# LilYau350/Variance-Aware-Weight

Hardware: AMD Instinct MI355X
Metric: training images/sec (higher is better)
Workload: dtype bf16; 1 GPU; DiT-B/4, 4x32x32 latents, 1000 classes; Trainer.train_step: q_sample + fwd + lambda-weighted MSE + bwd + AdamW + EMA; global batch 256 = 256 per GPU; global_batch=256, per_gpu_batch=256, parallelism=dp1, weight_type=lambda, hip_graph=False

## Files before the change

### include/vaw_hip.h

```cpp
#ifndef VAW_HIP_H
#define VAW_HIP_H
#include <stdint.h>

#ifdef __cplusplus
extern "C" {
#endif

typedef enum { VAW_OK = 0, VAW_ERR_INVALID = -1, VAW_ERR_LAUNCH = -2, VAW_ERR_UNSUPPORTED = -3 } vaw_status;
typedef enum { VAW_F32 = 0, VAW_BF16 = 1,
               VAW_FP8 = 2, VAW_BF8 = 3 ,
               VAW_F64 = 4  } vaw_dtype;
typedef void* vaw_stream;

int vaw_version(void);
const char* vaw_last_error_string(void);


int vaw_qsample_fwd(const float* x0, const float* noise, const int64_t* t, const float* tab_a, const float* tab_s,
                    int num_timesteps, float* x_t, int B, int64_t per_sample, vaw_stream stream);

int vaw_mix_rows(const float* x, const float* y, const float* ca, const float* cb, float* out, int B,
                 int64_t per_sample, vaw_stream stream);

int vaw_wmse_fwd(const float* model_out, const float* x0, const float* noise, const float* ca, const float* cb,
// ... 235 lines not shown
    int split;
    int xcd_parts;
    int grid_x, grid_y, grid_z, block;
    int64_t lds_bytes;
    int reduce;
    int rowsum_mode;
    int colsum_mode;
    int64_t colsum_rows;
    int64_t workspace_floats_used;
    int launches;
    int status;
} vaw_gemm_launch;
int vaw_gemm_plan(vaw_dtype dt, int a_kmajor, int b_kmajor, int64_t M, int64_t N, int64_t K, int64_t lda, int64_t ldb,
                  int64_t ldc, int64_t A, int64_t B, int64_t C, const vaw_epilogue* epi_host, int64_t workspace_floats,
                  const vaw_gemm_knobs* knobs, vaw_gemm_launch* out);

typedef struct {
    int epi_kind;
    int a_e5m2;
    int c_fp8, c_e5m2;
    int ntw;
    int tiles_m, tiles_n;
    int nk;
    int split;
    int grid, block;
    int64_t lds_bytes;
    int colsum_mode;
    int64_t colsum_rows;
    int64_t workspace_floats_used;
    int launches;
// ... 259 lines not shown
```

### variance-aware-weight_amd/_lib.py

```python
import ctypes as C
import os

import torch

_HERE = os.path.dirname(os.path.abspath(__file__))
LIB_PATH = os.environ.get("VAW_HIP_LIB") or os.path.join(_HERE, "libvaw_hip.so")

F32, BF16, FP8, BF8 = 0, 1, 2, 3
F64 = 4
TORCH_DTYPE = {F32: torch.float32, BF16: torch.bfloat16}

_p, _i, _l, _f, _d = C.c_void_p, C.c_int, C.c_int64, C.c_float, C.c_double


class Epilogue(C.Structure):
    _fields_ = [("bias", _p), ("act", _i), ("aux_in", _p), ("aux_out", _p), ("gate", _p), ("gate_ld", _l),
                ("resid", _p), ("rowadd", _p), ("rows_per_batch", _i), ("alpha", _f), ("beta", _f), ("out_f32", _i),
                ("colsum_out", _p), ("colsum_beta", _f), ("resid_is_act", _i), ("rowsum_a_out", _p), ("rowsum_a_beta", _f),
                ("colsum_partial_out", _p), ("colsum_rows_out", C.POINTER(C.c_int64))]


class AttnDesc(C.Structure):
    _fields_ = [("B", _i), ("H", _i), ("T", _i), ("hd", _i), ("q_sb", _l), ("q_sh", _l), ("q_st", _l), ("q_sd", _l),
                ("o_sb", _l), ("o_sh", _l), ("o_st", _l), ("o_sd", _l), ("scale", _f)]
# ... 25 lines not shown
                ("xcd_parts", _i), ("grid_x", _i), ("grid_y", _i), ("grid_z", _i), ("block", _i), ("lds_bytes", _l), ("reduce", _i),
                ("rowsum_mode", _i), ("colsum_mode", _i), ("colsum_rows", _l), ("workspace_floats_used", _l), ("launches", _i),
                ("status", _i)]


class Conv3x3Launch(C.Structure):
    _fields_ = [("variant", _i), ("ntw", _i), ("epi_kind", _i), ("transposed", _i), ("M", _l), ("N", _l), ("K", _l), ("split", _i),
                ("xcd_parts", _i), ("grid_x", _i), ("grid_y", _i), ("block", _i), ("lds_bytes", _l), ("reduce", _i), ("bias_grad", _i),
                ("colsum_mode", _i), ("colsum_rows", _l), ("workspace_floats_used", _l), ("launches", _i), ("status", _i)]


class GemmFp8Launch(C.Structure):
    _fields_ = [("epi_kind", _i), ("a_e5m2", _i), ("c_fp8", _i), ("c_e5m2", _i), ("ntw", _i), ("tiles_m", _i), ("tiles_n", _i), ("nk", _i),
                ("split", _i), ("grid", _i), ("block", _i), ("lds_bytes", _l), ("colsum_mode", _i), ("colsum_rows", _l),
                ("workspace_floats_used", _l), ("launches", _i), ("status", _i)]


class DitWsPlan(C.Structure):
    _fields_ = [("records", _i), ("colsum_sets", _i), ("own_dy", _i), ("Bk", _i), ("block_bytes", _l), ("block_stat_bytes", _l),
                ("shared_bytes", _l), ("colsum_bytes", _l), ("scratch_bytes", _l), ("cond_bytes", _l), ("total", _l)]


class CastColsumLaunch(C.Structure):
    _fields_ = [("grid_x", _i), ("block", _i), ("rows_per_lane", _i), ("bytes_read", _l), ("bytes_written", _l)]


ATTN_FWD, ATTN_BWD, ATTN_BWD_COLSUM = range(3)
(AV_ROWWISE, AV_FWD_T64, AV_FWD_G1, AV_FWD_G2, AV_FWD_BIG, AV_BWD_T64, AV_BWD_G1, AV_BWD_G2, AV_BWD_BIG_NT2,
 AV_BWD_BIG_NT4) = range(10)
AV_NAMES = ("rowwise", "fwd_t64", "fwd_g1", "fwd_g2", "fwd_big", "bwd_t64", "bwd_g1", "bwd_g2", "bwd_big_nt2", "bwd_big_nt4")
# ... 105 lines not shown
    "vaw_uncast_bf16": [_p, _p, _l, _f, _p],
    "vaw_wgrad_grouped": [_i, _i, _p, _l, _f, _p, _i, _p, _l, _p],
    "vaw_fp8_quantize": [_i, _i, _p, _l, _l, _l, _p, _l, _p, _l, _p, _p, _l, _p],
    "vaw_fp8_quantize_delayed": [_i, _i, _p, _l, _l, _l, _p, _l, _p, _l, _p, _p],
    "vaw_fp8_scale_update": [_p, _l, _p],
    "vaw_fp8_quantize_delayed_batched": [_i, _p, _p, _i, _p],
    "vaw_gemm_fp8": [_i, _l, _l, _l, _p, _l, _p, _p, _l, _p, _p, _l, C.POINTER(Epilogue), _p, _i, _p, _l, _p],
    "vaw_gemm_fp8_plan": [_i, _l, _l, _l, _l, _l, _l, _l, _l, _l, _l, _l, C.POINTER(Epilogue), _l, _i, _l, _l, _i, C.POINTER(GemmFp8Launch)],
    "vaw_fp8_transpose": [_p, _l, _l, _l, _p, _l, _p],
    "vaw_ln_modulate_fwd_fp8": [_p, _p, _p, _l, _p, _p, _i, _p, _p, _i, _i, _i, _f, _p],
    "vaw_gate_bwd_fp8": [_p, _p, _p, _l, _p, _p, _i, _p, _l, _p, _i, _i, _i, _p, _l, _p],
    "vaw_row_plan": [_i, _i, _l, _l, _l, _l, _l, _l, C.POINTER(RowLaunch)],
    "vaw_attn_plan": [_i, _i, C.POINTER(AttnDesc), _l, _l, _l, _l, _l, _l, _l, C.POINTER(AttnLaunch)],
    "vaw_gn_plan": [_i, _i, _i, _i, _i, _i, C.POINTER(GnLaunch)],
    "vaw_gemm_plan": [_i, _i, _i, _l, _l, _l, _l, _l, _l, _l, _l, _l, C.POINTER(Epilogue), _l, C.POINTER(GemmKnobs), C.POINTER(GemmLaunch)],
    "vaw_conv3x3_plan": [_i, _i, _l, _l, _l, _l, _i, _i, _i, _i, _i, C.POINTER(Epilogue), _l, _l, C.POINTER(GemmKnobs), _i, C.POINTER(Conv3x3Launch)],
    "vaw_dit_ws_plan": [_i, _i, _i, _i, _i, _i, _i, _i, _i, _i, _i, C.POINTER(DitWsPlan)],
    "vaw_latent_qsample": [_p, _p, _p, _p, _p, _p, _i, _f, _f, _p, _p, _p, _i, _l, _p],
    "vaw_wmse_fwd_t": [_p, _p, _p, _p, _p, _p, _p, _i, _p, _p, _f, _i, _l, _p],
    "vaw_wmse_bwd_t": [_p, _p, _p, _p, _p, _p, _p, _i, _p, _f, _p, _i, _l, _p],
    "vaw_ln_modulate_bwd_cast": [_i, _p, _p, _p, _p, _p, _l, _p, _p, _p, _p, _l, _i, _i, _i, _p, _l, _p, _p],
    "vaw_silu_bwd_cast": [_p, _p, _p, _p, _l, _p],
    "vaw_cast_colsum_plan": [_l, _l, _l, _l, _l, _l, _l, C.POINTER(CastColsumLaunch)],
    "vaw_cast_colsum_bf16": [_p, _l, _p, _l, _l, _l, _p, _f, _p],
    "vaw_row_sqnorms": [_p, _l, _i, _p, _p],
    "vaw_pairwise_ksmallest": [_p, _l, _p, _l, _i, _p, _p, _i, _p, _p, _l, _p],
    "vaw_ksmallest_merge": [_p, _l, _i, _i, _l, _l, _p, _p],
    "vaw_pairwise_within": [_p, _l, _p, _l, _i, _p, _p, _p, _i, _p, _i, _p, _p, _p],
    "vaw_pairwise_polysum": [_p, _l, _p, _l, _i, _p, _p, _i, _d, _d, _i, _i, _p, _p, _l, _p],
    "vaw_pairwise_count_within": [_p, _l, _p, _l, _i, _p, _p, _p, _i, _p, _p, _p, _l, _p],
# ... 64 lines not shown
        L.vaw_debug_force_generic_gemm.argtypes = [_i]
        L.vaw_debug_force_generic_gemm.restype = None
        L.vaw_debug_gemm_tile.argtypes = [_i]
        L.vaw_debug_gemm_tile.restype = None
        if hasattr(L, "vaw_gemm_default_knobs"):
            L.vaw_gemm_default_knobs.argtypes = [C.POINTER(GemmKnobs)]
            L.vaw_gemm_default_knobs.restype = None
        if hasattr(L, "vaw_debug_gn_flat"):
            L.vaw_debug_gn_flat.argtypes = [_i]
            L.vaw_debug_gn_flat.restype = None
        L.vaw_p8_set_reserved_cus.argtypes = [_i]
        L.vaw_p8_set_reserved_cus.restype = None
        if hasattr(L, "vaw_debug_wgrad_engine"):
            L.vaw_debug_wgrad_engine.argtypes = [_i]
            L.vaw_debug_wgrad_engine.restype = None
        L.vaw_debug_cu_hog.argtypes = [_i, _i, _p]
        L.vaw_debug_cu_hog.restype = _i
        _lib = L
    return _lib


def exported_symbols():
    return sorted(list(_PROTOS) + ["vaw_version", "vaw_last_error_string", "vaw_colsum_workspace_floats",
                                   "vaw_sumsq_workspace_floats", "vaw_groupnorm_workspace_floats", "vaw_wgrad_grouped_desc_bytes",
                                   "vaw_conv3x3_wgrad_small_workspace_floats", "vaw_row_bwd_workspace_floats",
                                   "vaw_fp8_quantize_workspace_floats", "vaw_p8_set_reserved_cus", "vaw_debug_wgrad_engine", "vaw_reduce_rows_batched_desc_bytes", "vaw_fp8_quantize_batched_desc_bytes",
                                   "vaw_gemm_default_knobs", "vaw_dropout_bits_words", "vaw_pairwise_workspace_bytes", "vaw_rk_partial_count",
                                   "vaw_pairwise_polysum_workspace_bytes", "vaw_pairwise_count_workspace_bytes"])


STEP_FUSED = os.environ.get("VAW_STEP_FUSED", "1") != "0"
ROWS_FWD_FUSED = os.environ.get("VAW_ROWS_FWD_FUSED", "1") != "0"


def check(rc, what):
    if rc != 0:
        raise VawError(f"{what} failed ({rc}): {lib().vaw_last_error_string().decode()}")


def stream_ptr():
    return torch.cuda.current_stream().cuda_stream
# ... 11 lines not shown
```

### variance-aware-weight_amd/csrc/gemm_plan.h

```cpp
#pragma once
#include "gemm_epi.h"

typedef vaw_gemm_knobs GemmKnobs;
GemmKnobs& vaw_gemm_knobs_state();
int vaw_p8_cus_available();

struct P8Plan {
    bool use;
    int ntw, split, grid;
};
P8Plan vaw_p8_plan(int64_t M, int64_t N, int64_t K, bool plain_f32, bool want_colsum, int64_t ws_floats, int force, int cus);

inline int pick_split(int64_t tiles, int64_t K, int64_t MN, int64_t ws_floats, bool plain_f32) {
    if (!plain_f32 || ws_floats <= 0) return 1;
    int64_t s = 512 / tiles;
    if (s > K / 256) s = K / 256;
    if (s > ws_floats / MN) s = ws_floats / MN;
    if (s > 64) s = 64;
    return s < 2 ? 1 : (int)s;
}
inline int no_empty_split(int nk, int split) {
    if (split <= 1) return 1;
    const int per = (nk + split - 1) / split;
    return (nk + per - 1) / per;
}

inline int xcd_parts_for(const GemmKnobs& k, int split) { return (k.xcdsplit && (split == 2 || split == 4 || split == 8)) ? 8 / split : 0; }

constexpr int64_t vaw_lds_t128(int bkt) { return (8 * 128 * bkt > 64 * 132 * 4 ? 8 * 128 * bkt : 64 * 132 * 4) + 4 * 128 * 4; }
constexpr int64_t vaw_lds_ring256() { return 4 * 4 * (128 * 32 * 2) + 8 * 256 * 4; }
constexpr int64_t vaw_lds_p8(int ntw) { return 2 * (4 + ntw) * 8192 + 32768; }
constexpr int64_t vaw_lds_sm(int mb, int nb, int stages) { return (int64_t)stages * (mb + nb) * 8192; }
constexpr int64_t vaw_lds_pd(int ntw) { return 3 * (2 + ntw) * 8192 + 8 * 2048; }
constexpr int64_t vaw_lds_ws(int ntw) { return 3 * (2 + ntw) * 8192; }
constexpr int64_t vaw_lds_generic() { return 2 * 16 * 144 * 4; }

inline EpiDev vaw_epi_dev(const vaw_epilogue* ep, const GemmKnobs& k) {
    EpiDev e{};
    e.alpha = 1.f;
    if (ep) {
        e.bias = ep->bias; e.act = ep->act; e.aux_in = ep->aux_in; e.aux_out = ep->aux_out; e.gate = ep->gate;
        e.gate_ld = ep->gate_ld; e.resid = ep->resid; e.rowadd = ep->rowadd; e.rpb = ep->rows_per_batch;
        e.alpha = ep->alpha; e.beta = ep->beta; e.out_f32 = ep->out_f32; e.resid_act = ep->resid_is_act;
    }
    if (e.rpb <= 0) e.rpb = 1;
    e.debug = k.debug;
// ... 4 lines not shown
```

### variance-aware-weight_amd/csrc/gemm_plan.hip

```cpp
#include <stdlib.h>

#include "gemm_plan.h"

extern "C" void vaw_gemm_default_knobs(vaw_gemm_knobs* k) {
    *k = vaw_gemm_knobs{};
    k->tile = -1;
    k->xcdsplit = k->epi = k->nt_aux = 1;
    k->sm_max_m = 8192;
    k->ws_loaders = 4;
    k->cus = 256;
}
GemmKnobs& vaw_gemm_knobs_state() {
    static GemmKnobs state = [] {
        static const struct { const char* env; int GemmKnobs::*field; } kEnv[] = {
            {"VAW_GEMM_BIG", &GemmKnobs::tile}, {"VAW_GEMM_BK", &GemmKnobs::bk}, {"VAW_GEMM_PD", &GemmKnobs::pd}, {"VAW_GEMM_WS", &GemmKnobs::ws},
            {"VAW_GEMM_XCDSPLIT", &GemmKnobs::xcdsplit}, {"VAW_SM_MAX_M", &GemmKnobs::sm_max_m}, {"VAW_SM_WIDE_M", &GemmKnobs::sm_wide_m},
            {"VAW_SM_NB", &GemmKnobs::sm_nb}, {"VAW_SM_STAGES", &GemmKnobs::sm_stages}, {"VAW_WS_LOADERS", &GemmKnobs::ws_loaders},
            {"VAW_GEMM_EPI", &GemmKnobs::epi}, {"VAW_GEMM_DEBUG", &GemmKnobs::debug}, {"VAW_P8_NT", &GemmKnobs::p8_nt}, {"VAW_P8_NT_AUX", &GemmKnobs::nt_aux}};
        GemmKnobs k;
        vaw_gemm_default_knobs(&k);
        for (const auto& e : kEnv)
            if (const char* v = getenv(e.env)) k.*e.field = atoi(v);
        k.ws_loaders = k.ws_loaders == 8 ? 8 : 4;
        k.p8_nt = k.p8_nt == 1;
// ... 219 lines not shown
    }
    const bool fused = p.rowsum_mode == VAW_GS_FUSED;
    p.reduce = p.split == 1 ? VAW_GR_NONE : !e.out_f32 ? VAW_GR_BF16 : fused ? VAW_GR_F32_ROWSUM : VAW_GR_F32;
    p.workspace_floats_used = (p.split > 1 ? (int64_t)p.split * M * N : 0) + (fused ? (int64_t)p.split * M : 0) +
                              (p.colsum_mode == VAW_GC_FOLD ? p.colsum_rows * N : 0);
    p.launches += (p.reduce != VAW_GR_NONE) + (fused && p.split == 1) + (p.colsum_mode == VAW_GC_FOLD);
    if (p.rowsum_mode == VAW_GS_SEPARATE && !a_kmajor && (rc = colsum_pass(p, dt, K, M, lda, A, ws)) != VAW_OK) return rc;
    if (p.colsum_mode == VAW_GC_SEPARATE && (rc = colsum_pass(p, e.out_f32 ? VAW_F32 : dt, M, N, ldc, C, ws)) != VAW_OK) return rc;
    *out = p;
    VAW_CHECK_ARG(!cs_part || p.colsum_rows <= *ep->colsum_rows_out, "gemm: colsum_partial_out holds %ld rows, this launch writes %ld",
                  (long)*ep->colsum_rows_out, (long)p.colsum_rows);
    VAW_CHECK_ARG(p.rowsum_mode != VAW_GS_SEPARATE || !a_kmajor, "gemm: rowsum_a_out is defined for a_kmajor = 0 (weight-gradient layout) only");
    VAW_CHECK_ARG(p.workspace_floats_used <= ws, "gemm: this launch needs a workspace of %ld floats, it has %ld", (long)p.workspace_floats_used,
                  (long)ws);
    out->status = p.status = VAW_OK;
    return VAW_OK;
}

extern "C" int vaw_conv3x3_plan(vaw_dtype dt, int mode, int64_t act, int64_t act2, int64_t w, int64_t out, int B, int H, int W, int Ci,
                                int Co, const vaw_epilogue* ep, int64_t workspace, int64_t ws, const vaw_gemm_knobs* knobs, int cus,
                                vaw_conv3x3_launch* plan) {
    VAW_CHECK_ARG(plan, "conv3x3_plan: plan is NULL");
    vaw_conv3x3_launch p = {};
    p.status = VAW_ERR_INVALID;
    p.epi_kind = -1;
    p.split = p.grid_y = 1;
    *plan = p;
    const GemmKnobs& k = knobs ? *knobs : vaw_gemm_knobs_state();
    if (cus <= 0) cus = k.cus > 0 ? k.cus : vaw_p8_cus_available();
    if (!workspace || ws < 0) ws = 0;
// ... 82 lines not shown
```

### variance-aware-weight_amd/dit.py

```python
import os

import numpy as np
import torch
import torch.nn as nn

from . import _lib as L
from . import ops
from ._lib import BF16, F32, ptr
from .flat import FlatModule

__all__ = ["DiT", "DiT_S", "DiT_B", "DiT_L", "DiT_XL", "DiT_models"]


def _sincos_1d(dim, pos):
    omega = 1.0 / 10000 ** (np.arange(dim // 2, dtype=np.float64) / (dim / 2.0))
    ang = np.einsum("m,d->md", pos.reshape(-1), omega)
    return np.concatenate([np.sin(ang), np.cos(ang)], axis=1)


def get_2d_sincos_pos_embed(dim, grid_size):
    gh = np.arange(grid_size, dtype=np.float32)
    gw = np.arange(grid_size, dtype=np.float32)
    grid = np.stack(np.meshgrid(gw, gh), axis=0).reshape([2, 1, grid_size, grid_size])
    return np.concatenate([_sincos_1d(dim // 2, grid[0]), _sincos_1d(dim // 2, grid[1])], axis=1)
# ... 493 lines not shown
        self._linear_fwd(ws, b, "f_xm2", None if fuse_rows else b["xm2"], pre + "mlp.fc1.", M, Dm, D, b["f_a"].epilogue_target() if fuse_a else ptr(b["a"]), Dm,
                         act=1, aux_out=ptr(b["hpre"]), **({"out_fp8": b["f_a"]} if fuse_a else {}))
        if rows_fc2:
            self._linear_fwd(ws, b, "f_a", b["a"], pre + "mlp.fc2.", M, D, Dm, ptr(b["y2"]), D)
            if recompute:
                return False
            sh, sc, out, mean, rstd = nxt if nxt is not None else (0, 0, 0, 0, 0)
            ops.gate_resid_ln_modulate_fwd(dt, ptr(b["y2"]), mo + 4 * 5 * D, ld, xmid, xout, sh, sc, ld, out, mean, rstd, B, T, D)
            return nxt is not None
        self._linear_fwd(ws, b, "f_a", None if fuse_a else b["a"], pre + "mlp.fc2.", M, D, Dm, xout, D, aux_out=ptr(b["y2"]),
                         gate=mo + 4 * 5 * D, gate_ld=ld, resid=xmid, rows_per_batch=T, out_f32=True)
        return False

    def _linear_fwd(self, ws, b, fkey, x, name, M, N, K, out, ldc, **epi):
        if not ws.fp8:
            ops.gemm(self._dt, 1, 1, M, N, K, ptr(x), K, self._w(name + "weight"), K, out, ldc, bias=self._p32(name + "bias"), **epi)
            return
        f = b[fkey].quantize(x, delayed=ws.d_fwd) if x is not None else b[fkey].transpose_from_q()
        w = self._fp8_w[name + "weight"]
        ops.gemm_fp8(M, N, K, f.last_q, K, ptr(f.scale), ptr(w.q), K, ptr(w.scale), out, ldc, bias=self._p32(name + "bias"), **epi)

    def _linear_dgrad(self, ws, b, fkey, dy, name, M, N, K, out, **epi):
        if not ws.fp8:
            ops.gemm(self._dt, 1, 0, M, K, N, ptr(dy) if isinstance(dy, torch.Tensor) else dy, N, self._w(name + "weight"), K, out, K, **epi)
            return
        f = b[fkey].quantize(dy, src_dt=BF16, delayed=ws.d_bwd) if dy is not None else b[fkey].transpose_from_q()
        w = self._fp8_w[name + "weight"]
        ops.gemm_fp8(M, K, N, f.last_q, N, ptr(f.scale), ptr(w.qt), N, ptr(w.scale), out, K, a_format=f.fmt, **epi)

    def _attn_desc(self, B):
        d = getattr(self, "_adesc", None)
        if d is None or d.B != B:
            d = self._adesc = ops.attn_desc_token_major(B, self.num_heads, self.T, self.D // self.num_heads)
        return d

    def _wgrad(self, dt, name, dy, x, Nw, Kw, M, beta, bias=True):
        ops.gemm(dt, 0, 0, Nw, Kw, M, dy, Nw, x, Kw, self._g(name + "weight"), Kw, beta=beta, out_f32=True,
                 rowsum_a_out=self._g(name + "bias") if bias else None, rowsum_a_beta=beta)

# ... 231 lines not shown
```

### variance-aware-weight_amd/ops.py

```python
import ctypes as C
import math

import numpy as np
import torch

from . import _lib as L
from ._lib import BF16, F32, AttnDesc, Epilogue, check, need_cuda, ptr, stream_ptr


def dt_of(t):
    if t.dtype == torch.float32:
        return F32
    if t.dtype == torch.bfloat16:
        return BF16
    raise L.VawError(f"unsupported activation dtype {t.dtype}")


def _f32c(*ts):
    for t in ts:
        if t is not None and (t.dtype != torch.float32 or not t.is_contiguous()):
            raise L.VawError(f"expected a contiguous float32 tensor, got {t.dtype} contiguous={t.is_contiguous()}")


def qsample(x0, noise, t, tab_a, tab_s):
# ... 550 lines not shown
                 epi.get("gate_ld", 0), epi.get("resid") or None, epi.get("rowadd") or None, epi.get("rows_per_batch", 0),
                 epi.get("alpha", 1.0), epi.get("beta", 0.0), 1 if epi.get("out_f32") else 0, epi.get("colsum_out") or None,
                 epi.get("colsum_beta", 0.0), 1 if epi.get("resid_is_act") else 0, epi.get("rowsum_a_out") or None,
                 epi.get("rowsum_a_beta", 0.0))
    rows = C.c_int64(colsum_partial_rows or 0)
    if colsum_partial_rows is not None:
        e.colsum_partial_out, e.colsum_rows_out = epi.get("colsum_partial_out", 16), C.pointer(rows)
    p = L.GemmLaunch()
    rc = L.lib().vaw_gemm_plan(dt, 1 if a_kmajor else 0, 1 if b_kmajor else 0, M, N, K, lda, ldb, ldc, A, B, Cp, C.byref(e),
                               workspace_floats, C.byref(knobs) if knobs is not None else None, C.byref(p))
    if check_status:
        check(rc, "vaw_gemm_plan")
    return p


def fp8_quantize(src_dt, src, R, C_, ld, q, qt, scale, fmt=L.FP8, device=None):
    ws = scratch_f32(device or torch.device("cuda", torch.cuda.current_device()), 0)
    check(L.lib().vaw_fp8_quantize(src_dt, fmt, src, R, C_, ld, q, C_, qt or None, R, scale, ws.data_ptr(), ws.numel(), stream_ptr()),
          "vaw_fp8_quantize")


FP8_MAX = {L.FP8: 448.0, L.BF8: 57344.0}


def fp8_states(formats, device, margin=2.0):
    st = torch.zeros(len(formats), 4)
    st[:, 0] = 1.0
    st[:, 2] = torch.tensor([FP8_MAX[f] / margin for f in formats])
    return st.to(device)

# ... 717 lines not shown
```

Baseline: 21330 images/sec.

## Add four-wave persistent bf16 Linear GEMM engine for large-K projections

```diff
diff --git a/include/vaw_hip.h b/include/vaw_hip.h
--- a/include/vaw_hip.h
+++ b/include/vaw_hip.h
@@ -273,6 +273,24 @@
 int vaw_gemm_plan(vaw_dtype dt, int a_kmajor, int b_kmajor, int64_t M, int64_t N, int64_t K, int64_t lda, int64_t ldb,
                   int64_t ldc, int64_t A, int64_t B, int64_t C, const vaw_epilogue* epi_host, int64_t workspace_floats,
                   const vaw_gemm_knobs* knobs, vaw_gemm_launch* out);
+
+typedef struct {
+    int tiles_m, tiles_n;
+    int nk;
+    int items, grid, block;
+    int64_t lds_bytes;
+    int has_bias;
+    int by_site;
+    int status;
+} vaw_linear4_launch;
+int vaw_linear4_plan(vaw_dtype dt, int a_kmajor, int b_kmajor, int64_t M, int64_t N, int64_t K, int64_t lda, int64_t ldb,
+                     int64_t ldc, int64_t A, int64_t B, int64_t C, const vaw_epilogue* epi_host, int cus, int engine,
+                     vaw_linear4_launch* out);
+int vaw_linear4(vaw_dtype dt, int a_kmajor, int b_kmajor, int64_t M, int64_t N, int64_t K, const void* A, int64_t lda,
+                const void* B, int64_t ldb, void* C, int64_t ldc, const vaw_epilogue* epi_host, vaw_stream stream);
+int vaw_linear_engine(void);
+void vaw_debug_linear_engine(int mode);
+void vaw_debug_linear4_last_launch(vaw_linear4_launch* out);
 
 typedef struct {
     int epi_kind;
diff --git a/variance-aware-weight_amd/_lib.py b/variance-aware-weight_amd/_lib.py
--- a/variance-aware-weight_amd/_lib.py
+++ b/variance-aware-weight_amd/_lib.py
@@ -63,6 +63,11 @@
     _fields_ = [("epi_kind", _i), ("a_e5m2", _i), ("c_fp8", _i), ("c_e5m2", _i), ("ntw", _i), ("tiles_m", _i), ("tiles_n", _i), ("nk", _i),
                 ("split", _i), ("grid", _i), ("block", _i), ("lds_bytes", _l), ("colsum_mode", _i), ("colsum_rows", _l),
                 ("workspace_floats_used", _l), ("launches", _i), ("status", _i)]
+
+
+class Linear4Launch(C.Structure):
+    _fields_ = [("tiles_m", _i), ("tiles_n", _i), ("nk", _i), ("items", _i), ("grid", _i), ("block", _i), ("lds_bytes", _l),
+                ("has_bias", _i), ("by_site", _i), ("status", _i)]
 
 
 class DitWsPlan(C.Structure):
@@ -198,6 +203,8 @@
     "vaw_attn_plan": [_i, _i, C.POINTER(AttnDesc), _l, _l, _l, _l, _l, _l, _l, C.POINTER(AttnLaunch)],
     "vaw_gn_plan": [_i, _i, _i, _i, _i, _i, C.POINTER(GnLaunch)],
     "vaw_gemm_plan": [_i, _i, _i, _l, _l, _l, _l, _l, _l, _l, _l, _l, C.POINTER(Epilogue), _l, C.POINTER(GemmKnobs), C.POINTER(GemmLaunch)],
+    "vaw_linear4_plan": [_i, _i, _i, _l, _l, _l, _l, _l, _l, _l, _l, _l, C.POINTER(Epilogue), _i, _i, C.POINTER(Linear4Launch)],
+    "vaw_linear4": [_i, _i, _i, _l, _l, _l, _p, _l, _p, _l, _p, _l, C.POINTER(Epilogue), _p],
     "vaw_conv3x3_plan": [_i, _i, _l, _l, _l, _l, _i, _i, _i, _i, _i, C.POINTER(Epilogue), _l, _l, C.POINTER(GemmKnobs), _i, C.POINTER(Conv3x3Launch)],
     "vaw_dit_ws_plan": [_i, _i, _i, _i, _i, _i, _i, _i, _i, _i, _i, C.POINTER(DitWsPlan)],
     "vaw_latent_qsample": [_p, _p, _p, _p, _p, _p, _i, _f, _f, _p, _p, _p, _i, _l, _p],
@@ -292,6 +299,13 @@
         if hasattr(L, "vaw_debug_wgrad_engine"):
             L.vaw_debug_wgrad_engine.argtypes = [_i]
             L.vaw_debug_wgrad_engine.restype = None
+        if hasattr(L, "vaw_debug_linear_engine"):
+            L.vaw_debug_linear_engine.argtypes = [_i]
+            L.vaw_debug_linear_engine.restype = None
+            L.vaw_linear_engine.argtypes = []
+            L.vaw_linear_engine.restype = _i
+            L.vaw_debug_linear4_last_launch.argtypes = [C.POINTER(Linear4Launch)]
+            L.vaw_debug_linear4_last_launch.restype = None
         L.vaw_debug_cu_hog.argtypes = [_i, _i, _p]
         L.vaw_debug_cu_hog.restype = _i
         _lib = L
@@ -302,7 +316,7 @@
     return sorted(list(_PROTOS) + ["vaw_version", "vaw_last_error_string", "vaw_colsum_workspace_floats",
                                    "vaw_sumsq_workspace_floats", "vaw_groupnorm_workspace_floats", "vaw_wgrad_grouped_desc_bytes",
                                    "vaw_conv3x3_wgrad_small_workspace_floats", "vaw_row_bwd_workspace_floats",
-                                   "vaw_fp8_quantize_workspace_floats", "vaw_p8_set_reserved_cus", "vaw_debug_wgrad_engine", "vaw_reduce_rows_batched_desc_bytes", "vaw_fp8_quantize_batched_desc_bytes",
+                                   "vaw_fp8_quantize_workspace_floats", "vaw_p8_set_reserved_cus", "vaw_debug_wgrad_engine", "vaw_debug_linear_engine", "vaw_linear_engine", "vaw_debug_linear4_last_launch", "vaw_reduce_rows_batched_desc_bytes", "vaw_fp8_quantize_batched_desc_bytes",
                                    "vaw_gemm_default_knobs", "vaw_dropout_bits_words", "vaw_pairwise_workspace_bytes", "vaw_rk_partial_count",
                                    "vaw_pairwise_polysum_workspace_bytes", "vaw_pairwise_count_workspace_bytes"])
 
diff --git a/variance-aware-weight_amd/csrc/gemm_l4.hip b/variance-aware-weight_amd/csrc/gemm_l4.hip
--- /dev/null
+++ b/variance-aware-weight_amd/csrc/gemm_l4.hip
@@ -0,0 +1,36 @@
+#include "gemm_l4_kernel.h"
+#include "gemm_plan.h"
+static_assert(L4_LDS_BYTES == vaw_lds_l4(), "gemm_plan.h: LDS size of the four-wave Linear engine");
+
+static int g_linear_engine = -2;
+extern "C" int vaw_linear_engine(void) {
+    if (g_linear_engine == -2) {
+        const char* v = getenv("VAW_LINEAR_ENGINE");
+        const int m = v ? atoi(v) : -1;
+        g_linear_engine = (m == 0 || m == 1) ? m : -1;
+    }
+    return g_linear_engine;
+}
+extern "C" void vaw_debug_linear_engine(int mode) { g_linear_engine = (mode == 0 || mode == 1) ? mode : -1; }
+
+static vaw_linear4_launch g_last_launch = {};
+extern "C" void vaw_debug_linear4_last_launch(vaw_linear4_launch* out) { if (out) *out = g_last_launch; }
+
+extern "C" int vaw_linear4(vaw_dtype dt, int a_kmajor, int b_kmajor, int64_t M, int64_t N, int64_t K, const void* A, int64_t lda,
+                           const void* B, int64_t ldb, void* C, int64_t ldc, const vaw_epilogue* ep, vaw_stream stream) {
+    vaw_linear4_launch p;
+    const int rc = vaw_linear4_plan(dt, a_kmajor, b_kmajor, M, N, K, lda, ldb, ldc, (int64_t)(uintptr_t)A, (int64_t)(uintptr_t)B,
+                                    (int64_t)(uintptr_t)C, ep, 0, -2, &p);
+    if (rc) return rc;
+    const float alpha = ep ? ep->alpha : 1.f;
+    const float* bias = ep ? ep->bias : nullptr;
+    const int nt_off = !vaw_gemm_knobs_state().p8_nt;
+    hipStream_t s = (hipStream_t)stream;
+    VAW_CHECK_ARG(p.block == 256 && p.lds_bytes == L4_LDS_BYTES, "linear4: the plan's block %d / LDS %ld are not the kernel's", p.block, (long)p.lds_bytes);
+    const int block = p.block, lds = (int)p.lds_bytes;
+    if (b_kmajor) l4_launch_one<true>((const bf16_t*)A, lda, (const bf16_t*)B, ldb, p.nk, p.tiles_m, p.tiles_n, p.grid, block, lds, (bf16_t*)C, ldc, (int)M, (int)N, alpha, bias, nt_off, s);
+    else l4_launch_one<false>((const bf16_t*)A, lda, (const bf16_t*)B, ldb, p.nk, p.tiles_m, p.tiles_n, p.grid, block, lds, (bf16_t*)C, ldc, (int)M, (int)N, alpha, bias, nt_off, s);
+    VAW_CHECK_LAUNCH("linear4");
+    g_last_launch = p;
+    return VAW_OK;
+}
diff --git a/variance-aware-weight_amd/csrc/gemm_l4_kernel.h b/variance-aware-weight_amd/csrc/gemm_l4_kernel.h
--- /dev/null
+++ b/variance-aware-weight_amd/csrc/gemm_l4_kernel.h
@@ -0,0 +1,295 @@
+#pragma once
+#include "gemm_p8_kernel.h"
+
+#define L4_BN 192
+#define L4_STAGE (7 * P8_PART)
+#define L4_EPI_BYTES (4 * 4096)
+#define L4_LDS_BYTES (2 * L4_STAGE + L4_EPI_BYTES)
+static_assert(L4_STAGE == P8Cfg<3>::stage_bytes && L4_BN == P8Cfg<3>::BN, "the stage layout and tile width of gemm_p8_kernel<.., 3, ..>");
+static_assert(L4_LDS_BYTES <= 160 * 1024, "LDS of one CU");
+static_assert(4 * P8_PART + (96 + 15) * 128 + 7 * 16 + 5 * 2048 + 16 <= L4_STAGE, "the last k-major B fragment read ends inside its stage");
+static_assert(3 * P8_PART + 2048 < 65536 && 5 * 2048 < 65536 && 4096 + 512 < 65536, "fragment reads address through the 16-bit DS offset");
+
+template <int OFF>
+__device__ __forceinline__ bf16x8 l4_frag_k(unsigned addr) {
+    bf16x8 v;
+    asm volatile("ds_read_b128 %0, %1 offset:%2" : "=&v"(v) : "v"(addr), "i"(OFF) : "memory");
+    return v;
+}
+template <int OFF>
+__device__ __forceinline__ bf16x8 l4_frag_mn(unsigned addr) {
+    bf16x4 lo, hi;
+    asm volatile("ds_read_b64_tr_b16 %0, %2 offset:%3\n\tds_read_b64_tr_b16 %1, %2 offset:%4"
+                 : "=&v"(lo), "=&v"(hi)
+                 : "v"(addr), "i"(OFF), "i"(OFF + 512)
+                 : "memory");
+    return bf16x8{lo[0], lo[1], lo[2], lo[3], hi[0], hi[1], hi[2], hi[3]};
+}
+
+#define L4_SB() __builtin_amdgcn_sched_barrier(0)
+#define L4_IC(v) std::integral_constant<int, (v)>{}
+
+template <bool BKM>
+__global__ void __launch_bounds__(256) __attribute__((amdgpu_waves_per_eu(1, 1)))
+gemm_l4_kernel(const bf16_t* __restrict__ A, int64_t lda, const bf16_t* __restrict__ B, int64_t ldb, int nk, int tiles_m, int tiles_n,
+               bf16_t* __restrict__ C, int64_t ldc, int M, int N, float alpha, const float* __restrict__ bias, int nt_off) {
+    constexpr int BN = L4_BN;
+    extern __shared__ __attribute__((aligned(16))) char smem[];
+    const int lane = threadIdx.x & 63;
+    const int wid = __builtin_amdgcn_readfirstlane(threadIdx.x >> 6);
+    const int wr = wid >> 1, wc = wid & 1;
+    const int G = gridDim.x;
+    const int n_items = tiles_m * tiles_n;
+    int it_cur;
+    {
+        const int b = blockIdx.x, x = b & 7, q = G >> 3, r = G & 7;
+        it_cur = (x < r ? x * (q + 1) : r * (q + 1) + (x - r) * q) + (b >> 3);
+    }
+    if (it_cur >= n_items) return;
+    auto decode = [&](int tile, int& tm, int& tn) __attribute__((always_inline)) {
+        if (tiles_n >= 8) {
+            const int gsz = 4 * tiles_n, gi = tile / gsz, within = tile - gi * gsz;
+            const int rows = tiles_m - 4 * gi < 4 ? tiles_m - 4 * gi : 4;
+            tn = within / rows;
+            tm = 4 * gi + within - tn * rows;
+        } else {
+            tm = tile / tiles_n;
+            tn = tile - tm * tiles_n;
+        }
+    };
+
+    int iss_item = it_cur, iss_kt = 0, iss_stage = 0;
+    bool iss_done = false;
+    __amdgpu_buffer_rsrc_t rs_a = epi_rsrc(A), rs_b = epi_rsrc(B);
+    unsigned so_a = 0, so_b = 0;
+    const unsigned step_a = 128, step_b = BKM ? 128u : (unsigned)(64 * ldb * 2);
+    u32x4_t off_a0 = {0, 0, 0, 0}, off_a1 = {0, 0, 0, 0};
+    u32x4_t off_b0 = {0, 0, 0, 0}, off_b1 = {0, 0, 0, 0};
+    auto iss_open = [&]() __attribute__((always_inline)) {
+        int tm, tn;
+        decode(iss_item, tm, tn);
+        int lane = threadIdx.x & 63;
+        asm volatile("" : "+v"(lane));
+        iss_kt = 0;
+        const int64_t m0 = (int64_t)tm * P8_BM, n0 = (int64_t)tn * BN;
+        const int mvalid = M - m0 < P8_BM ? (int)(M - m0) : P8_BM;
+        so_a = so_b = 0;
+        rs_a = epi_rsrc((const char*)A + m0 * lda * 2);
+        rs_b = epi_rsrc((const char*)B + (BKM ? n0 * ldb : n0) * 2);
+        off_a0 = u32x4_t{p8_src_off<true>(true, 0, wid, lane, lda, mvalid), p8_src_off<true>(true, 1, wid, lane, lda, mvalid),
+                         p8_src_off<true>(true, 2, wid, lane, lda, mvalid), p8_src_off<true>(true, 3, wid, lane, lda, mvalid)};
+        off_a1 = u32x4_t{p8_src_off<true>(true, 0, 4 + wid, lane, lda, mvalid), p8_src_off<true>(true, 1, 4 + wid, lane, lda, mvalid),
+                         p8_src_off<true>(true, 2, 4 + wid, lane, lda, mvalid), p8_src_off<true>(true, 3, 4 + wid, lane, lda, mvalid)};
+        off_b0 = u32x4_t{p8_src_off<BKM>(false, 0, wid, lane, ldb, BN), p8_src_off<BKM>(false, 1, wid, lane, ldb, BN),
+                         p8_src_off<BKM>(false, 2, wid, lane, ldb, BN), 0u};
+        off_b1 = u32x4_t{p8_src_off<BKM>(false, 0, 4 + wid, lane, ldb, BN), p8_src_off<BKM>(false, 1, 4 + wid, lane, ldb, BN),
+                         p8_src_off<BKM>(false, 2, 4 + wid, lane, ldb, BN), 0u};
+    };
+    auto iss_close = [&]() __attribute__((always_inline)) {
+        off_a0 = off_a1 = off_b0 = off_b1 = u32x4_t{EPI_OOB, EPI_OOB, EPI_OOB, EPI_OOB};
+    };
+    auto iss_a = [&](auto cc) __attribute__((always_inline)) {
+        constexpr int c = decltype(cc)::value, p = c >> 1;
+        char* dst = smem + iss_stage * L4_STAGE + p * P8_PART + ((c & 1) * 4 + wid) * 1024;
+        p8_dma16(rs_a, dst, (c & 1) ? off_a1[p] : off_a0[p], so_a);
+    };
+    auto iss_b = [&](auto cc) __attribute__((always_inline)) {
+        constexpr int c = decltype(cc)::value, p = c >> 1;
+        char* dst = smem + iss_stage * L4_STAGE + (4 + p) * P8_PART + ((c & 1) * 4 + wid) * 1024;
+        p8_dma16(rs_b, dst, (c & 1) ? off_b1[p] : off_b0[p], so_b);
+    };
+    auto iss_advance = [&]() __attribute__((always_inline)) {
+        iss_stage ^= 1;
+        if (iss_done) return;
+        so_a += step_a;
+        so_b += step_b;
+        if (++iss_kt == nk) {
+            iss_item += G;
+            if (iss_item >= n_items) { iss_done = true; iss_close(); }
+            else iss_open();
+        }
+    };
+
+    unsigned rA[2], rB[BKM ? 2 : 6];
+    {
+        const unsigned base = (unsigned)(uintptr_t)(lds_ptr_t)smem;
+        const int li = lane & 15;
+#pragma unroll
+        for (int s = 0; s < 2; ++s) {
+            const unsigned lane_off = base + li * 128 + ((((lane >> 4) + 4 * s) ^ (li >> 1)) << 4);
+            rA[s] = lane_off + wr * 32 * 128;
+            if (BKM) rB[s] = lane_off + 4 * P8_PART + wc * 96 * 128;
+        }
+        if (!BKM) {
+            const int q = li >> 2, p = li & 3;
+            const int kb0 = 8 * (lane >> 4) + q, swz = p8_mn_swz(kb0);
+            const unsigned lane_off = base + 4 * P8_PART + kb0 * 128 + ((p >> 1) << 4) + 8 * (p & 1);
+#pragma unroll
+            for (int u = 0; u < 6; ++u) {
+                const int n = wc * 96 + 16 * u;
+                rB[u] = lane_off + (n >> 6) * P8_PART + (((2 * ((n & 63) >> 4)) ^ swz) << 4);
+            }
+        }
+    }
+    int rd_delta = L4_STAGE;
+    bf16x8 fa[2][8], fb[2][6];
+    auto read_a = [&](auto nxc, auto ic) __attribute__((always_inline)) {
+        constexpr int nx = decltype(nxc)::value, i = decltype(ic)::value;
+        fa[nx][i] = l4_frag_k<(i >> 1) * P8_PART + (i & 1) * 2048>(rA[nx]);
+    };
+    auto read_b = [&](auto nxc, auto uc) __attribute__((always_inline)) {
+        constexpr int nx = decltype(nxc)::value, u = decltype(uc)::value;
+        if constexpr (BKM) fb[nx][u] = l4_frag_k<u * 2048>(rB[nx]);
+        else fb[nx][u] = l4_frag_mn<nx * 4096>(rB[u]);
+    };
+
+    iss_open();
+    iss_a(L4_IC(0)); iss_a(L4_IC(1)); iss_a(L4_IC(2)); iss_a(L4_IC(3)); iss_a(L4_IC(4)); iss_a(L4_IC(5)); iss_a(L4_IC(6)); iss_a(L4_IC(7));
+    iss_b(L4_IC(0)); iss_b(L4_IC(1)); iss_b(L4_IC(2)); iss_b(L4_IC(3)); iss_b(L4_IC(4)); iss_b(L4_IC(5));
+    iss_advance();
+    iss_a(L4_IC(0)); iss_a(L4_IC(1)); iss_a(L4_IC(2)); iss_a(L4_IC(3)); iss_a(L4_IC(4)); iss_a(L4_IC(5)); iss_a(L4_IC(6)); iss_a(L4_IC(7));
+    iss_b(L4_IC(0)); iss_b(L4_IC(1)); iss_b(L4_IC(2));
+    asm volatile("s_waitcnt vmcnt(11)" ::: "memory");
+    __builtin_amdgcn_s_barrier();
+    L4_SB();
+    read_a(L4_IC(0), L4_IC(0)); read_a(L4_IC(0), L4_IC(1)); read_a(L4_IC(0), L4_IC(2)); read_a(L4_IC(0), L4_IC(3));
+    read_a(L4_IC(0), L4_IC(4)); read_a(L4_IC(0), L4_IC(5)); read_a(L4_IC(0), L4_IC(6)); read_a(L4_IC(0), L4_IC(7));
+    read_b(L4_IC(0), L4_IC(0)); read_b(L4_IC(0), L4_IC(1)); read_b(L4_IC(0), L4_IC(2));
+    read_b(L4_IC(0), L4_IC(3)); read_b(L4_IC(0), L4_IC(4)); read_b(L4_IC(0), L4_IC(5));
+    L4_SB();
+
+    for (; it_cur < n_items; it_cur += G) {
+        int tm, tn;
+        decode(it_cur, tm, tn);
+        const int64_t m0 = (int64_t)tm * P8_BM, n0 = (int64_t)tn * BN;
+        f32x4 acc[8][6];
+#pragma unroll
+        for (int i = 0; i < 8; ++i)
+#pragma unroll
+            for (int u = 0; u < 6; ++u) acc[i][u] = f32x4{0, 0, 0, 0};
+        auto step = [&](auto sc, auto uc) __attribute__((always_inline)) {
+            constexpr int s = decltype(sc)::value, u = decltype(uc)::value, nx = s ^ 1;
+            if constexpr (u == 0) { if constexpr (BKM) asm volatile("s_waitcnt lgkmcnt(5)" ::: "memory"); else asm volatile("s_waitcnt lgkmcnt(10)" ::: "memory"); }
+            if constexpr (u == 1) { if constexpr (BKM) asm volatile("s_waitcnt lgkmcnt(8)" ::: "memory"); else asm volatile("s_waitcnt lgkmcnt(12)" ::: "memory"); }
+            if constexpr (u == 2) { if constexpr (BKM) asm volatile("s_waitcnt lgkmcnt(11)" ::: "memory"); else asm volatile("s_waitcnt lgkmcnt(14)" ::: "memory"); }
+            L4_SB();
+#define L4_MMA(i) acc[i][u] = __builtin_amdgcn_mfma_f32_16x16x32_bf16(fb[s][u], fa[s][i], acc[i][u], 0, 0, 0)
+            L4_MMA(0);
+            L4_SB();
+            if constexpr (u == 0) { read_a(L4_IC(nx), L4_IC(0)); read_a(L4_IC(nx), L4_IC(1)); }
+            if constexpr (u == 1) { read_a(L4_IC(nx), L4_IC(4)); read_a(L4_IC(nx), L4_IC(5)); }
+            if constexpr (u >= 3) read_b(L4_IC(nx), L4_IC(2 * (u - 3)));
+            L4_SB();
+            L4_MMA(1);
+            L4_MMA(2);
+            L4_SB();
+            if constexpr (u == 0) { read_a(L4_IC(nx), L4_IC(2)); read_a(L4_IC(nx), L4_IC(3)); }
+            if constexpr (u == 1) { read_a(L4_IC(nx), L4_IC(6)); read_a(L4_IC(nx), L4_IC(7)); }
+            if constexpr (u >= 3) read_b(L4_IC(nx), L4_IC(2 * (u - 3) + 1));
+            L4_SB();
+            L4_MMA(3);
+            L4_MMA(4);
+            L4_SB();
+            if constexpr (s == 0 && u < 3) iss_b(L4_IC(3 + u));
+            if constexpr (s == 0 && u == 3) { iss_a(L4_IC(0)); iss_a(L4_IC(1)); }
+            if constexpr (s == 0 && u > 3) iss_a(L4_IC(u - 2));
+            if constexpr (s == 1 && u == 0) { iss_a(L4_IC(4)); iss_a(L4_IC(5)); }
+            if constexpr (s == 1 && u > 0 && u < 3) iss_a(L4_IC(5 + u));
+            if constexpr (s == 1 && u >= 3) iss_b(L4_IC(u - 3));
+            L4_SB();
+            L4_MMA(5);
+            L4_MMA(6);
+            L4_MMA(7);
+#undef L4_MMA
+            L4_SB();
+        };
+        for (int kt = 0; kt < nk; ++kt) {
+            step(L4_IC(0), L4_IC(0)); step(L4_IC(0), L4_IC(1)); step(L4_IC(0), L4_IC(2));
+            iss_advance();
+            asm volatile("s_waitcnt vmcnt(6) lgkmcnt(0)" ::: "memory");
+            __builtin_amdgcn_s_barrier();
+            L4_SB();
+            step(L4_IC(0), L4_IC(3)); step(L4_IC(0), L4_IC(4)); step(L4_IC(0), L4_IC(5));
+#pragma unroll
+            for (int s = 0; s < 2; ++s) rA[s] += rd_delta;
+#pragma unroll
+            for (int k = 0; k < (BKM ? 2 : 6); ++k) rB[k] += rd_delta;
+            rd_delta = -rd_delta;
+            step(L4_IC(1), L4_IC(0)); step(L4_IC(1), L4_IC(1)); step(L4_IC(1), L4_IC(2));
+            asm volatile("s_waitcnt vmcnt(8) lgkmcnt(0)" ::: "memory");
+            __builtin_amdgcn_s_barrier();
+            L4_SB();
+            step(L4_IC(1), L4_IC(3)); step(L4_IC(1), L4_IC(4)); step(L4_IC(1), L4_IC(5));
+        }
+        asm volatile("s_waitcnt lgkmcnt(0)\n\ts_nop 15" ::: "memory");
+        L4_SB();
+
+        char* ep = smem + 2 * L4_STAGE + wid * 4096;
+        int lane_e = lane;
+        asm volatile("" : "+v"(lane_e));
+        const int wr_row = lane_e & 15, wr_g = lane_e >> 4;
+        const int rd_row = lane_e >> 3, rd_c8 = lane_e & 7;
+        const unsigned ep_base = (unsigned)(uintptr_t)(lds_ptr_t)ep;
+        const unsigned ep_w = ep_base + wr_row * 256 + ((wr_g ^ (wr_row & 3)) << 4);
+        unsigned ep_r[2];
+#pragma unroll
+        for (int pass = 0; pass < 2; ++pass) {
+            const int rr = pass * 8 + rd_row;
+            ep_r[pass] = ep_base + rr * 256 + (((2 * rd_c8) ^ rr) << 4);
+        }
+        const int64_t m_last = (int64_t)M - 1;
+        const __amdgpu_buffer_rsrc_t rs_c = epi_rsrc(C + m0 * ldc + n0);
+        const int64_t mrow0 = m0 + wr * 128 + rd_row;
+#pragma unroll
+        for (int hh = 0; hh < 2; ++hh) {
+            const int nu = hh == 0 ? 4 : 2;
+            const int wn0 = wc * 96 + 64 * hh;
+            const int64_t n = n0 + wn0 + 8 * rd_c8;
+            const bool col_ok = 8 * rd_c8 < 16 * nu && n < N;
+            const int64_t n_ld = col_ok ? n : n0;
+            const int loc_col = wn0 + 8 * rd_c8;
+            f32x4 b0 = {0, 0, 0, 0}, b1 = {0, 0, 0, 0};
+            if (bias) {
+                b0 = load4(bias + n_ld);
+                b1 = load4(bias + n_ld + 4);
+                asm volatile("" ::"v"(b0), "v"(b1));
+            }
+#pragma unroll
+            for (int i = 0; i < 8; ++i) {
+#pragma unroll
+                for (int u = 0; u < 4; ++u)
+                    if (u < nu) asm volatile("ds_write_b128 %0, %1" ::"v"(ep_w + (unsigned)(((4 * u) ^ (wr_row & 12)) << 4)), "a"(acc[i][4 * hh + (u < nu ? u : 0)]) : "memory");
+#pragma unroll
+                for (int pass = 0; pass < 2; ++pass) {
+                    const int k = 2 * i + pass;
+                    const int64_t m = mrow0 + 8 * k;
+                    f32x4 v0, v1;
+                    asm volatile("ds_read_b128 %0, %2\n\tds_read_b128 %1, %3\n\ts_waitcnt lgkmcnt(0)"
+                                 : "=&v"(v0), "=&v"(v1)
+                                 : "v"(ep_r[pass]), "v"(ep_r[pass] ^ 16u)
+                                 : "memory");
+                    L4_SB();
+                    const bool ok = col_ok && m <= m_last;
+                    const int loc = (int)((m - m0) * ldc) + loc_col;
+                    v0 = v0 * alpha + b0;
+                    v1 = v1 * alpha + b1;
+                    const bf16x8 r = {(bf16_t)v0[0], (bf16_t)v0[1], (bf16_t)v0[2], (bf16_t)v0[3], (bf16_t)v1[0], (bf16_t)v1[1], (bf16_t)v1[2], (bf16_t)v1[3]};
+                    buf_store16(rs_c, ok ? 2u * (unsigned)loc : EPI_OOB, r, !nt_off);
+                    L4_SB();
+                }
+            }
+        }
+    }
+    asm volatile("s_waitcnt vmcnt(0) lgkmcnt(0)" ::: "memory");
+}
+
+template <bool BKM>
+static void l4_launch_one(const bf16_t* a, int64_t lda, const bf16_t* b, int64_t ldb, int nk, int tiles_m, int tiles_n, int grid, int block,
+                          int lds, bf16_t* c, int64_t ldc, int M, int N, float alpha, const float* bias, int nt_off, hipStream_t s) {
+    static bool attr_done = false;
+    if (!attr_done) {
+        (void)hipFuncSetAttribute((const void*)gemm_l4_kernel<BKM>, hipFuncAttributeMaxDynamicSharedMemorySize, L4_LDS_BYTES);
+        attr_done = true;
+    }
+    gemm_l4_kernel<BKM><<<grid, block, lds, s>>>(a, lda, b, ldb, nk, tiles_m, tiles_n, c, ldc, M, N, alpha, bias, nt_off);
+}
diff --git a/variance-aware-weight_amd/csrc/gemm_plan.h b/variance-aware-weight_amd/csrc/gemm_plan.h
--- a/variance-aware-weight_amd/csrc/gemm_plan.h
+++ b/variance-aware-weight_amd/csrc/gemm_plan.h
@@ -3,6 +3,7 @@
 
 typedef vaw_gemm_knobs GemmKnobs;
 GemmKnobs& vaw_gemm_knobs_state();
+extern "C" int vaw_linear_engine(void);
 int vaw_p8_cus_available();
 
 struct P8Plan {
@@ -30,6 +31,7 @@
 constexpr int64_t vaw_lds_t128(int bkt) { return (8 * 128 * bkt > 64 * 132 * 4 ? 8 * 128 * bkt : 64 * 132 * 4) + 4 * 128 * 4; }
 constexpr int64_t vaw_lds_ring256() { return 4 * 4 * (128 * 32 * 2) + 8 * 256 * 4; }
 constexpr int64_t vaw_lds_p8(int ntw) { return 2 * (4 + ntw) * 8192 + 32768; }
+constexpr int64_t vaw_lds_l4() { return 2 * (4 + 3) * 8192 + 4 * 4096; }
 constexpr int64_t vaw_lds_sm(int mb, int nb, int stages) { return (int64_t)stages * (mb + nb) * 8192; }
 constexpr int64_t vaw_lds_pd(int ntw) { return 3 * (2 + ntw) * 8192 + 8 * 2048; }
 constexpr int64_t vaw_lds_ws(int ntw) { return 3 * (2 + ntw) * 8192; }
diff --git a/variance-aware-weight_amd/csrc/gemm_plan.hip b/variance-aware-weight_amd/csrc/gemm_plan.hip
--- a/variance-aware-weight_amd/csrc/gemm_plan.hip
+++ b/variance-aware-weight_amd/csrc/gemm_plan.hip
@@ -257,6 +257,61 @@
     VAW_CHECK_ARG(p.workspace_floats_used <= ws, "gemm: this launch needs a workspace of %ld floats, it has %ld", (long)p.workspace_floats_used,
                   (long)ws);
     out->status = p.status = VAW_OK;
+    return VAW_OK;
+}
+
+#define L4_REFUSE(cond, ...)                       \
+    do {                                           \
+        if (cond) {                                \
+            vaw_set_error(__VA_ARGS__);            \
+            out->status = VAW_ERR_UNSUPPORTED;     \
+            return VAW_ERR_UNSUPPORTED;            \
+        }                                          \
+    } while (0)
+static bool l4_site_measured(bool b_kmajor, int64_t items, int64_t K, int cus) {
+    (void)b_kmajor;
+    return items <= cus && K >= 2304;
+}
+extern "C" int vaw_linear4_plan(vaw_dtype dt, int a_kmajor, int b_kmajor, int64_t M, int64_t N, int64_t K, int64_t lda, int64_t ldb,
+                                int64_t ldc, int64_t A, int64_t B, int64_t C, const vaw_epilogue* ep, int cus, int engine,
+                                vaw_linear4_launch* out) {
+    VAW_CHECK_ARG(out, "linear4_plan: out is NULL");
+    *out = vaw_linear4_launch{};
+    out->status = VAW_ERR_INVALID;
+    VAW_CHECK_ARG(M > 0 && N > 0 && K > 0 && A && B && C, "linear4: bad sizes M=%ld N=%ld K=%ld or a NULL operand", (long)M, (long)N, (long)K);
+    if (cus <= 0) cus = vaw_p8_cus_available();
+    if (engine < -1 || engine > 1) engine = vaw_linear_engine();
+    L4_REFUSE(dt != VAW_BF16, "linear4: bf16 operands only (dtype %d)", (int)dt);
+    L4_REFUSE(!a_kmajor, "linear4: A must be k-major ([M][K])");
+    L4_REFUSE(M < 256, "linear4: M = %ld is below one 256-row tile", (long)M);
+    L4_REFUSE(N % 192 != 0, "linear4: N = %ld is not a multiple of the 192-column tile", (long)N);
+    L4_REFUSE(K % 64 != 0 || K < 1024, "linear4: K = %ld must be a multiple of 64 and at least 1024", (long)K);
+    L4_REFUSE(M >= (1LL << 31) || N >= (1LL << 31), "linear4: M, N must fit 31 bits");
+    L4_REFUSE(lda < K || ldb < (b_kmajor ? K : N) || ldc < N, "linear4: leading dimension too small");
+    L4_REFUSE(lda % 8 != 0 || ldb % 8 != 0 || ldc % 8 != 0, "linear4: leading dimensions must be multiples of 8 elements (16 bytes)");
+    L4_REFUSE(((A | B | C) & 15) != 0, "linear4: A, B and C must be 16-byte aligned");
+    if (ep) {
+        L4_REFUSE(ep->act != 0 || ep->aux_out || ep->gate || ep->resid || ep->rowadd, "linear4: the epilogue is a plain store with an optional bias");
+        L4_REFUSE(ep->out_f32 || ep->beta != 0.f, "linear4: bf16 output with beta = 0 only");
+        L4_REFUSE(ep->colsum_out || ep->colsum_partial_out || ep->rowsum_a_out, "linear4: no fused column or row sums");
+        L4_REFUSE(((uintptr_t)ep->bias & 15) != 0, "linear4: the bias must be 16-byte aligned");
+    }
+    const int64_t lim = 1LL << 31;
+    L4_REFUSE(512 * lda + 2 * K >= lim || (b_kmajor ? 384 * ldb + 2 * K : 2 * K * ldb + 384) >= lim || 512 * ldc + 384 >= lim,
+              "linear4: a tile's operands or output span 2 GiB or more");
+    const int64_t tiles_m = (M + 255) / 256, tiles_n = N / 192, items = tiles_m * tiles_n;
+    L4_REFUSE(items >= (1LL << 30), "linear4: too many tiles");
+    L4_REFUSE(engine != 1 && items < cus / 2, "linear4: %ld items leave more than half of %d CUs idle", (long)items, cus);
+    out->tiles_m = (int)tiles_m;
+    out->tiles_n = (int)tiles_n;
+    out->nk = (int)(K / 64);
+    out->items = (int)items;
+    out->grid = (int)(items < cus ? items : cus);
+    out->block = 256;
+    out->lds_bytes = vaw_lds_l4();
+    out->has_bias = ep && ep->bias ? 1 : 0;
+    out->by_site = l4_site_measured(b_kmajor != 0, items, K, cus) ? 1 : 0;
+    out->status = VAW_OK;
     return VAW_OK;
 }
 
diff --git a/variance-aware-weight_amd/dit.py b/variance-aware-weight_amd/dit.py
--- a/variance-aware-weight_amd/dit.py
+++ b/variance-aware-weight_amd/dit.py
@@ -531,7 +531,11 @@
 
     def _linear_fwd(self, ws, b, fkey, x, name, M, N, K, out, ldc, **epi):
         if not ws.fp8:
-            ops.gemm(self._dt, 1, 1, M, N, K, ptr(x), K, self._w(name + "weight"), K, out, ldc, bias=self._p32(name + "bias"), **epi)
+            w, bias = self._w(name + "weight"), self._p32(name + "bias")
+            if ops.linear4_wanted(self._dt, 1, M, N, K, ptr(x), K, w, K, out, ldc, bias=bias, **epi):
+                ops.linear4(self._dt, 1, 1, M, N, K, ptr(x), K, w, K, out, ldc, bias=bias)
+            else:
+                ops.gemm(self._dt, 1, 1, M, N, K, ptr(x), K, w, K, out, ldc, bias=bias, **epi)
             return
         f = b[fkey].quantize(x, delayed=ws.d_fwd) if x is not None else b[fkey].transpose_from_q()
         w = self._fp8_w[name + "weight"]
@@ -539,7 +543,11 @@
 
     def _linear_dgrad(self, ws, b, fkey, dy, name, M, N, K, out, **epi):
         if not ws.fp8:
-            ops.gemm(self._dt, 1, 0, M, K, N, ptr(dy) if isinstance(dy, torch.Tensor) else dy, N, self._w(name + "weight"), K, out, K, **epi)
+            dyp, w = ptr(dy) if isinstance(dy, torch.Tensor) else dy, self._w(name + "weight")
+            if ops.linear4_wanted(self._dt, 0, M, K, N, dyp, N, w, K, out, K, **epi):
+                ops.linear4(self._dt, 1, 0, M, K, N, dyp, N, w, K, out, K)
+            else:
+                ops.gemm(self._dt, 1, 0, M, K, N, dyp, N, w, K, out, K, **epi)
             return
         f = b[fkey].quantize(dy, src_dt=BF16, delayed=ws.d_bwd) if dy is not None else b[fkey].transpose_from_q()
         w = self._fp8_w[name + "weight"]
diff --git a/variance-aware-weight_amd/ops.py b/variance-aware-weight_amd/ops.py
--- a/variance-aware-weight_amd/ops.py
+++ b/variance-aware-weight_amd/ops.py
@@ -588,6 +588,54 @@
     return p
 
 
+def linear4_plan(dt, a_kmajor, b_kmajor, M, N, K, A, lda, B, ldb, Cp, ldc, *, cus=0, engine=-2, check_status=False, **epi):
+    e = Epilogue(epi.get("bias") or None, epi.get("act", 0), epi.get("aux_in") or None, epi.get("aux_out") or None, epi.get("gate") or None,
+                 epi.get("gate_ld", 0), epi.get("resid") or None, epi.get("rowadd") or None, epi.get("rows_per_batch", 0),
+                 epi.get("alpha", 1.0), epi.get("beta", 0.0), 1 if epi.get("out_f32") else 0, epi.get("colsum_out") or None,
+                 epi.get("colsum_beta", 0.0), 1 if epi.get("resid_is_act") else 0, epi.get("rowsum_a_out") or None,
+                 epi.get("rowsum_a_beta", 0.0))
+    if epi.get("colsum_partial") is not None or epi.get("colsum_partial_out"):
+        e.colsum_partial_out = epi.get("colsum_partial_out") or 16
+    p = L.Linear4Launch()
+    rc = L.lib().vaw_linear4_plan(dt, 1 if a_kmajor else 0, 1 if b_kmajor else 0, M, N, K, lda, ldb, ldc, A, B, Cp, C.byref(e), cus, engine, C.byref(p))
+    if check_status:
+        check(rc, "vaw_linear4_plan")
+    return p
+
+
+def linear4(dt, a_kmajor, b_kmajor, M, N, K, A, lda, B, ldb, Cp, ldc, *, bias=None, alpha=1.0):
+    e = Epilogue(bias or None, 0, None, None, None, 0, None, None, 0, alpha, 0.0, 0, None, 0.0, 0, None, 0.0)
+    tr = gemm_trace
+    if tr is not None:
+        e0, e1 = tr.events()
+        e0.record()
+    check(L.lib().vaw_linear4(dt, 1 if a_kmajor else 0, 1 if b_kmajor else 0, M, N, K, A, lda, B, ldb, Cp, ldc, C.byref(e), stream_ptr()),
+          "vaw_linear4")
+    if tr is not None:
+        e1.record()
+        tr.add(1, bool(a_kmajor), bool(b_kmajor), M, N, K, e0, e1, float(2 * (M * K + N * K + M * N)))
+
+
+def linear_engine(mode=None):
+    if mode is not None:
+        L.lib().vaw_debug_linear_engine(int(mode))
+    return int(L.lib().vaw_linear_engine())
+
+
+def linear4_wanted(dt, b_kmajor, M, N, K, A, lda, B, ldb, Cp, ldc, **epi):
+    mode = linear_engine()
+    if mode == 0 or dt != BF16:
+        return False
+    p = linear4_plan(dt, 1, b_kmajor, M, N, K, A, lda, B, ldb, Cp, ldc, **epi)
+    if p.status != 0 or mode == 1:
+        return p.status == 0
+    if not p.by_site:
+        return False
+    ws_n = scratch_f32(torch.device("cuda", torch.cuda.current_device()), 0).numel() if (not epi.get("bias") and K >= 2048) else 0
+    g = gemm_plan(dt, 1, b_kmajor, M, N, K, A, lda, B, ldb, Cp, ldc, workspace_floats=ws_n, check_status=False, **epi)
+    return g.status == 0 and g.variant == L.GV_PERSISTENT and g.ntw == 3 and g.epi_kind == L.P8_STORE and g.split == 1
+
+
 def fp8_quantize(src_dt, src, R, C_, ld, q, qt, scale, fmt=L.FP8, device=None):
     ws = scratch_f32(device or torch.device("cuda", torch.cuda.current_device()), 0)
     check(L.lib().vaw_fp8_quantize(src_dt, fmt, src, R, C_, ld, q, C_, qt or None, R, scale, ws.data_ptr(), ws.numel(), stream_ptr()),
```

New measurement: 21280 images/sec. About the same (-0.2%).
